# skypilot-org/skypilot

Hardware: AMD Instinct MI355X
Metric: tokens/sec (node) sky-launched Llama-3-8B (higher is better)
Workload: dtype bf16; 1 GPU; model=llama3-8b, global_batch=6, seq_len=4096, parallelism=dp1, sky_launched=True

## Files before the change

skypilot_amd/ops/csrc/attention_bwd.hip:

```cpp
#include <cstdlib>
#include "common.h"

#define ATT_D 128
#define BM 64
#define BN 64

extern "C" __global__ void attn_bwd_pre_kernel(
    const unsigned short* __restrict__ dO, const unsigned short* __restrict__ O,
    float* __restrict__ Dvec, long long rows, int Hq) {
  (void)Hq;
  const int lane = threadIdx.x & 63;
  const long long wave_id =
      (long long)blockIdx.x * (blockDim.x >> 6) + (threadIdx.x >> 6);
  const long long stride = (long long)gridDim.x * (blockDim.x >> 6);
  for (long long row = wave_id; row < rows; row += stride) {
    const unsigned short* drow = dO + row * ATT_D;
    const unsigned short* orow = O + row * ATT_D;
    float acc = bf2f(drow[lane]) * bf2f(orow[lane]) +
                bf2f(drow[lane + 64]) * bf2f(orow[lane + 64]);
    acc = wave_reduce_sum(acc);
    if (lane == 0) Dvec[row] = acc;
  }
}

extern "C" __global__ __launch_bounds__(256, 2) void attn_bwd_dkv_kernel(
    const unsigned short* __restrict__ Q, const unsigned short* __restrict__ K,
    const unsigned short* __restrict__ V, const unsigned short* __restrict__ dO,
    const float* __restrict__ lse, const float* __restrict__ Dvec,
    unsigned short* __restrict__ dK, unsigned short* __restrict__ dV, int B,
    int S, int Hq, int Hkv, float scale, int causal) {
  __shared__ unsigned short q_lds[BM * ATT_D];
  __shared__ unsigned short qt_lds[ATT_D * BM];
  __shared__ unsigned short do_lds[BM * ATT_D];
  __shared__ unsigned short dot_lds[ATT_D * BM];
  __shared__ unsigned short p_lds[BN * BM];
  __shared__ unsigned short ds_lds[BN * BM];
// ... 28 lines not shown
    }
  }

  f32x4 dv_acc[8], dk_acc[8];
#pragma unroll
  for (int ct = 0; ct < 8; ++ct) {
    dv_acc[ct] = f32x4{0.f, 0.f, 0.f, 0.f};
    dk_acc[ct] = f32x4{0.f, 0.f, 0.f, 0.f};
  }

  for (int g = 0; g < group; ++g) {
    const int qh = kvh * group + g;
    const unsigned short* Qb = Q + ((long long)b * S * Hq + qh) * ATT_D;
    const unsigned short* dOb = dO + ((long long)b * S * Hq + qh) * ATT_D;
    const float* lse_b = lse + ((long long)b * Hq + qh) * S;
    const float* dvec_b = Dvec + (long long)b * S * Hq + qh;

    const int qt0 = causal ? kvbase / BM : 0;
    for (int qt = qt0; qt < S / BM; ++qt) {
      const int qbase = qt * BM;
      __syncthreads();
#pragma unroll
      for (int i = 0; i < 4; ++i) {
        int ch = (tid & 7) | ((i & 1) << 3);
        int row = (tid >> 3) | ((i >> 1) << 5);
        s16x8 qv = *(const s16x8*)(Qb + (long long)(qbase + row) * q_rowstride + ch * 8);
        *(s16x8*)((char*)q_lds + swz(row * 256 + ch * 16, row)) = qv;
        s16x8 dov = *(const s16x8*)(dOb + (long long)(qbase + row) * q_rowstride + ch * 8);
        *(s16x8*)((char*)do_lds + swz(row * 256 + ch * 16, row)) = dov;
#pragma unroll
        for (int j = 0; j < 8; ++j) {
// ... 16 lines not shown
          int qrow = ct * 16 + lrow;
          s16x8 bq = *(const s16x8*)((char*)q_lds +
                                     swz(qrow * 256 + (ks * 32 + lgrp * 8) * 2, qrow));
          st[ct] = MFMA_BF16(as_bf16x8(a_k[ks]), as_bf16x8(bq), st[ct]);
          s16x8 bdo = *(const s16x8*)((char*)do_lds +
                                      swz(qrow * 256 + (ks * 32 + lgrp * 8) * 2, qrow));
          dpt[ct] = MFMA_BF16(as_bf16x8(a_v[ks]), as_bf16x8(bdo), dpt[ct]);
        }
      }

      const int my_kvrow = kvbase + 16 * w + lgrp * 4;
#pragma unroll
      for (int ct = 0; ct < 4; ++ct) {
        int qcol = qbase + ct * 16 + lrow;
        float l = lse_b[qcol];
        float dv = dvec_b[(long long)qcol * Hq];
#pragma unroll
        for (int r = 0; r < 4; ++r) {
          float sv = st[ct][r] * scale;
          float pv;
          if ((causal && qcol < my_kvrow + r) || l == -INFINITY)
            pv = 0.f;
          else
            pv = __expf(sv - l);
          int prow = 16 * w + lgrp * 4 + r;
          int pcol = ct * 16 + lrow;
          int off = swzP(prow * 128 + pcol * 2, prow);
          *(unsigned short*)((char*)p_lds + off) = f2bf_trunc(pv);
          *(unsigned short*)((char*)ds_lds + off) =
              f2bf(pv * (dpt[ct][r] - dv));
        }
// ... 54 lines not shown
  const int qbase = qt * BM;

  const int tid = threadIdx.x;
  const int lane = tid & 63;
  const int w = tid >> 6;
  const int lrow = lane & 15;
  const int lgrp = lane >> 4;

  const long long q_rowstride = (long long)Hq * ATT_D;
  const long long kv_rowstride = (long long)Hkv * ATT_D;
  const unsigned short* Qb = Q + ((long long)b * S * Hq + qh) * ATT_D;
  const unsigned short* Kb = K + ((long long)b * S * Hkv + kvh) * ATT_D;
  const unsigned short* Vb = V + ((long long)b * S * Hkv + kvh) * ATT_D;
  const unsigned short* dOb = dO + ((long long)b * S * Hq + qh) * ATT_D;
  const float* lse_b = lse + ((long long)b * Hq + qh) * S;
  const float* dvec_b = Dvec + (long long)b * S * Hq + qh;

  s16x8 a_q[4], a_do[4];
  float my_lse[4], my_dvec[4];
  {
    const int qrow = qbase + 16 * w + lrow;
    const unsigned short* qsrc = Qb + (long long)qrow * q_rowstride;
    const unsigned short* dsrc = dOb + (long long)qrow * q_rowstride;
#pragma unroll
    for (int ks = 0; ks < 4; ++ks) {
      a_q[ks] = *(const s16x8*)(qsrc + ks * 32 + lgrp * 8);
      a_do[ks] = *(const s16x8*)(dsrc + ks * 32 + lgrp * 8);
    }
#pragma unroll
    for (int r = 0; r < 4; ++r) {
      int rr = qbase + 16 * w + lgrp * 4 + r;
      my_lse[r] = lse_b[rr];
      my_dvec[r] = dvec_b[(long long)rr * Hq];
    }
  }

  f32x4 dq_acc[8];
#pragma unroll
  for (int ct = 0; ct < 8; ++ct) dq_acc[ct] = f32x4{0.f, 0.f, 0.f, 0.f};

  const int n_kv_tiles = causal ? (qbase + BM + BN - 1) / BN : S / BN;
  for (int kt = 0; kt < n_kv_tiles; ++kt) {
    const int kvbase = kt * BN;
    __syncthreads();
#pragma unroll
    for (int i = 0; i < 4; ++i) {
      int ch = (tid & 7) | ((i & 1) << 3);
      int row = (tid >> 3) | ((i >> 1) << 5);
// ... 124 lines not shown
  }

  f32x16 dv_acc, dk_acc;
#pragma unroll
  for (int r = 0; r < 16; ++r) {
    dv_acc[r] = 0.f;
    dk_acc[r] = 0.f;
  }

  for (int g = 0; g < group; ++g) {
    const int qh_head = kvh_head * group + g;
    const unsigned short* Qb = Q + ((long long)b * S * Hq + qh_head) * ATT_D;
    const unsigned short* dOb =
        dO + ((long long)b * S * Hq + qh_head) * ATT_D;
    const float* lse_b = lse + ((long long)b * Hq + qh_head) * S;
    const float* dvec_b = Dvec + (long long)b * S * Hq + qh_head;

    const int qt0 = causal ? kvbase / BM : 0;
    for (int qt = qt0; qt < S / BM; ++qt) {
      const int qbase = qt * BM;
      __syncthreads();
#pragma unroll
      for (int i2 = 0; i2 < 2; ++i2) {
        int i = i2 * 2 + (tid >> 8);
        int t = tid & 255;
        int ch = (t & 7) | ((i & 1) << 3);
        int row = (t >> 3) | ((i >> 1) << 5);
        s16x8 qv = *(const s16x8*)(Qb + (long long)(qbase + row) *
                                       q_rowstride + ch * 8);
        *(s16x8*)((char*)q_lds + swz(row * 256 + ch * 16, row)) = qv;
        s16x8 dov = *(const s16x8*)(dOb + (long long)(qbase + row) *
// ... 32 lines not shown
          if ((causal && qcol < kvbase + kvrow) || l == -INFINITY)
            pv = 0.f;
          else
            pv = __expf(acc[r] * scale - l);
          int prow = kvrow;
          int pcol = t_qh * 32 + col;
          *(unsigned short*)((char*)p_lds +
                             swzP(prow * 128 + pcol * 2, prow)) =
              f2bf_trunc(pv);
        }
      }
      __syncthreads();

      if (!is_st) {
        const int qcol = qbase + t_qh * 32 + col;
        const float dvq = dvec_b[(long long)qcol * Hq];
#pragma unroll
        for (int r = 0; r < 16; ++r) {
          int kvrow = t_kvh * 32 + (r & 3) + 8 * (r >> 2) + 4 * half;
          int off = swzP(kvrow * 128 + (t_qh * 32 + col) * 2, kvrow);
          float pv = bf2f(*(const unsigned short*)((char*)p_lds + off));
          *(unsigned short*)((char*)ds_lds + off) =
              f2bf(pv * (acc[r] - dvq));
        }
      }
#pragma unroll
      for (int ks = 0; ks < 4; ++ks) {
        int arow = o_kvh * 32 + col;
        s16x8 afrag = *(const s16x8*)(
            (char*)p_lds +
            swzP(arow * 128 + (ks * 16 + half * 8) * 2, arow));
// ... 29 lines not shown
    dKb[(long long)kvrow * kv_rowstride + d] = f2bf(dk_acc[r] * scale);
    dVb[(long long)kvrow * kv_rowstride + d] = f2bf(dv_acc[r]);
  }
}

extern "C" __global__ void attn_bwd_dkv_tr_kernel(
    const unsigned short*, const unsigned short*, const unsigned short*,
    const unsigned short*, const float*, const float*, unsigned short*,
    unsigned short*, int, int, int, int, float, int);

extern "C" void attn_bwd_v3_launch(const void* Q, const void* K,
                                   const void* V, const void* dO,
                                   const float* lse, const float* Dvec,
                                   void* dQ, void* dK, void* dV, int B,
                                   int S, int Hq, int Hkv, float scale,
                                   bool causal, hipStream_t stream);

extern "C" __global__ void attn_bwd_dkv_swapped_kernel(
    const unsigned short*, const unsigned short*, const unsigned short*,
    const unsigned short*, const float*, const float*, unsigned short*,
    unsigned short*, int, int, int, int, float, int);

extern "C" __global__ void attn_bwd_dq_swapped_kernel(
    const unsigned short*, const unsigned short*, const unsigned short*,
    const unsigned short*, const float*, const float*, unsigned short*,
    int, int, int, int, float, int);

extern "C" void attn_bwd_launch(const void* Q, const void* K, const void* V,
                                const void* O, const void* dO,
                                const float* lse, float* Dvec, void* dQ,
                                void* dK, void* dV, int B, int S, int Hq,
                                int Hkv, float scale, bool causal,
                                hipStream_t stream) {
  long long rows = (long long)B * S * Hq;
  hipLaunchKernelGGL(attn_bwd_pre_kernel, dim3(membound_grid(rows, 4)),
                     dim3(256), 0, stream, (const unsigned short*)dO,
                     (const unsigned short*)O, Dvec, rows, Hq);
  static const int use_bwd_v3 = [] {
    const char* e = getenv("SKY_ATTN_BWD_V3");
    return e ? atoi(e) : 1;
  }();
  if (use_bwd_v3 && S % 128 == 0) {
    attn_bwd_v3_launch(Q, K, V, dO, lse, Dvec, dQ, dK, dV, B, S, Hq, Hkv,
                       scale, causal, stream);
    return;
  }
  static const int dkv_swapped = [] {
    const char* e = getenv("SKY_ATTN_DKV_SWAPPED");
    return e ? atoi(e) : 0;
  }();
  static const int dkv_tr = [] {
    const char* e = getenv("SKY_ATTN_DKV_TR");
    return e ? atoi(e) : 0;
  }();
  if (dkv_tr)
    hipLaunchKernelGGL(attn_bwd_dkv_tr_kernel, dim3(S / BN, B * Hkv),
                       dim3(256), 0, stream, (const unsigned short*)Q,
                       (const unsigned short*)K, (const unsigned short*)V,
                       (const unsigned short*)dO, lse, Dvec,
// ... 51 lines not shown
  const int qbase = qt * BM;

  const int tid = threadIdx.x;
  const int lane = tid & 63;
  const int w = tid >> 6;
  const int lrow = lane & 15;
  const int lgrp = lane >> 4;

  const long long q_rowstride = (long long)Hq * ATT_D;
  const long long kv_rowstride = (long long)Hkv * ATT_D;
  const unsigned short* Qb = Q + ((long long)b * S * Hq + qh) * ATT_D;
  const unsigned short* Kb = K + ((long long)b * S * Hkv + kvh) * ATT_D;
  const unsigned short* Vb = V + ((long long)b * S * Hkv + kvh) * ATT_D;
  const unsigned short* dOb = dO + ((long long)b * S * Hq + qh) * ATT_D;
  const float* lse_b = lse + ((long long)b * Hq + qh) * S;
  const float* dvec_b = Dvec + (long long)b * S * Hq + qh;

  s16x8 q_b[4], do_b[4];
  const int my_q = qbase + 16 * w + lrow;
  {
    const unsigned short* qsrc = Qb + (long long)my_q * q_rowstride;
    const unsigned short* dsrc = dOb + (long long)my_q * q_rowstride;
#pragma unroll
    for (int ks = 0; ks < 4; ++ks) {
      q_b[ks] = *(const s16x8*)(qsrc + ks * 32 + lgrp * 8);
      do_b[ks] = *(const s16x8*)(dsrc + ks * 32 + lgrp * 8);
    }
  }
  const float my_lse = lse_b[my_q];
  const float my_dvec = dvec_b[(long long)my_q * Hq];

  f32x4 dq_t[8];
#pragma unroll
  for (int ct = 0; ct < 8; ++ct) dq_t[ct] = f32x4{0.f, 0.f, 0.f, 0.f};

  const int n_kv_tiles = causal ? (qbase + BM + BN - 1) / BN : S / BN;
  for (int kt = 0; kt < n_kv_tiles; ++kt) {
    const int kvbase = kt * BN;
    __syncthreads();
#pragma unroll
    for (int i = 0; i < 4; ++i) {
      int ch = (tid & 7) | ((i & 1) << 3);
      int row = (tid >> 3) | ((i >> 1) << 5);
      s16x8 kv8 = *(const s16x8*)(Kb + (long long)(kvbase + row) * kv_rowstride + ch * 8);
      *(s16x8*)((char*)k_lds + swz(row * 256 + ch * 16, row)) = kv8;
// ... 117 lines not shown
    }
  }

  f32x4 dv_t[8], dk_t[8];
#pragma unroll
  for (int ct = 0; ct < 8; ++ct) {
    dv_t[ct] = f32x4{0.f, 0.f, 0.f, 0.f};
    dk_t[ct] = f32x4{0.f, 0.f, 0.f, 0.f};
  }

  for (int g = 0; g < group; ++g) {
    const int qh = kvh * group + g;
    const unsigned short* Qb = Q + ((long long)b * S * Hq + qh) * ATT_D;
    const unsigned short* dOb = dO + ((long long)b * S * Hq + qh) * ATT_D;
    const float* lse_b = lse + ((long long)b * Hq + qh) * S;
    const float* dvec_b = Dvec + (long long)b * S * Hq + qh;

    const int qt0 = causal ? kvbase / BM : 0;
    for (int qt = qt0; qt < S / BM; ++qt) {
      const int qbase = qt * BM;
      __syncthreads();
#pragma unroll
      for (int i = 0; i < 4; ++i) {
        int ch = (tid & 7) | ((i & 1) << 3);
        int row = (tid >> 3) | ((i >> 1) << 5);
        s16x8 qv = *(const s16x8*)(Qb + (long long)(qbase + row) * q_rowstride + ch * 8);
        *(s16x8*)((char*)q_lds + swz(row * 256 + ch * 16, row)) = qv;
        s16x8 dov = *(const s16x8*)(dOb + (long long)(qbase + row) * q_rowstride + ch * 8);
        *(s16x8*)((char*)do_lds + swz(row * 256 + ch * 16, row)) = dov;
#pragma unroll
        for (int j = 0; j < 8; ++j) {
// ... 20 lines not shown
          s16x8 a_q = *(const s16x8*)((char*)q_lds +
              swz(qrow * 256 + (ks * 32 + lgrp * 8) * 2, qrow));
          sp[qsub] = MFMA_BF16(as_bf16x8(a_q), as_bf16x8(k_b[ks]),
                               sp[qsub]);
          s16x8 a_do = *(const s16x8*)((char*)do_lds +
              swz(qrow * 256 + (ks * 32 + lgrp * 8) * 2, qrow));
          dp[qsub] = MFMA_BF16(as_bf16x8(a_do), as_bf16x8(v_b[ks]),
                               dp[qsub]);
        }

      float lse_l[4], dv_l[4];
#pragma unroll
      for (int qsub = 0; qsub < 4; ++qsub) {
        int qc = qbase + qsub * 16 + lrow;
        lse_l[qsub] = lse_b[qc];
        dv_l[qsub] = dvec_b[(long long)qc * Hq];
      }
#pragma unroll
      for (int qsub = 0; qsub < 4; ++qsub)
#pragma unroll
        for (int r = 0; r < 4; ++r) {
          int qrow = qbase + qsub * 16 + lgrp * 4 + r;
          float l = __shfl(lse_l[qsub], lgrp * 4 + r, 64);
          float pv;
          if ((causal && qrow < my_kv) || l == -INFINITY)
            pv = 0.f;
          else
            pv = __expf(sp[qsub][r] * scale - l);
          sp[qsub][r] = pv;
          dp[qsub][r] = pv * (dp[qsub][r] -
                              __shfl(dv_l[qsub], lgrp * 4 + r, 64));
// ... 90 lines not shown
  f32x4 dv_acc[8], dk_acc[8];
#pragma unroll
  for (int ct = 0; ct < 8; ++ct) {
    dv_acc[ct] = f32x4{0.f, 0.f, 0.f, 0.f};
    dk_acc[ct] = f32x4{0.f, 0.f, 0.f, 0.f};
  }

  const unsigned int q_base_a = (unsigned int)(unsigned long long)q_lds;
  const unsigned int do_base_a = (unsigned int)(unsigned long long)do_lds;

  for (int g = 0; g < group; ++g) {
    const int qh = kvh * group + g;
    const unsigned short* Qb = Q + ((long long)b * S * Hq + qh) * ATT_D;
    const unsigned short* dOb = dO + ((long long)b * S * Hq + qh) * ATT_D;
    const float* lse_b = lse + ((long long)b * Hq + qh) * S;
    const float* dvec_b = Dvec + (long long)b * S * Hq + qh;

    const int qt0 = causal ? kvbase / BM : 0;
    for (int qt = qt0; qt < S / BM; ++qt) {
      const int qbase = qt * BM;
      __syncthreads();
#pragma unroll
      for (int i = 0; i < 4; ++i) {
        int idx = tid + i * 256;
        int row = idx >> 4, ch = idx & 15;
        s16x8 qv = *(const s16x8*)(Qb + (long long)(qbase + row) * q_rowstride + ch * 8);
        *(s16x8*)((char*)q_lds + swz(row * 256 + ch * 16, row)) = qv;
        s16x8 dov = *(const s16x8*)(dOb + (long long)(qbase + row) * q_rowstride + ch * 8);
        *(s16x8*)((char*)do_lds + swz(row * 256 + ch * 16, row)) = dov;
      }
      __syncthreads();
// ... 8 lines not shown
          int qrow = ct * 16 + lrow;
          s16x8 bq = *(const s16x8*)((char*)q_lds +
                                     swz(qrow * 256 + (ks * 32 + lgrp * 8) * 2, qrow));
          st[ct] = MFMA_BF16(as_bf16x8(a_k[ks]), as_bf16x8(bq), st[ct]);
          s16x8 bdo = *(const s16x8*)((char*)do_lds +
                                      swz(qrow * 256 + (ks * 32 + lgrp * 8) * 2, qrow));
          dpt[ct] = MFMA_BF16(as_bf16x8(a_v[ks]), as_bf16x8(bdo), dpt[ct]);
        }
      }

      const int my_kvrow = kvbase + 16 * w + lgrp * 4;
#pragma unroll
      for (int ct = 0; ct < 4; ++ct) {
        int qcol = qbase + ct * 16 + lrow;
        float l = lse_b[qcol];
        float dvv = dvec_b[(long long)qcol * Hq];
#pragma unroll
        for (int r = 0; r < 4; ++r) {
          float sv = st[ct][r] * scale;
          float pv;
          if ((causal && qcol < my_kvrow + r) || l == -INFINITY)
            pv = 0.f;
          else
            pv = __expf(sv - l);
          int prow = 16 * w + lgrp * 4 + r;
          int pcol = ct * 16 + lrow;
          int off = swzP(prow * 128 + pcol * 2, prow);
          *(unsigned short*)((char*)p_lds + off) = f2bf_trunc(pv);
          *(unsigned short*)((char*)ds_lds + off) =
              f2bf(pv * (dpt[ct][r] - dvv));
        }
// ... 71 lines not shown
```

skypilot_amd/ops/csrc/attention_bwd_v3.hip:

```cpp
#include <cstdlib>

#include "attn_v3.h"

#define ATT_D 128

__device__ __forceinline__ int vsubz(int q, int d) {
  return (((q >> 2) << 3) + ((d >> 4) ^ ((q >> 2) & 7))) * 64 +
         ((q & 3) << 4) + (d & 15);
}

extern "C" __global__ __launch_bounds__(256, 2) void attn_bwd_dkv_v3_kernel(
    const unsigned short* __restrict__ Q, const unsigned short* __restrict__ K,
    const unsigned short* __restrict__ V, const unsigned short* __restrict__ dO,
    const float* __restrict__ lse, const float* __restrict__ Dvec,
    unsigned short* __restrict__ dK, unsigned short* __restrict__ dV, int B,
    int S, int Hq, int Hkv, float scale, int causal) {
  __shared__ unsigned short q_lds[32 * ATT_D];
  __shared__ unsigned short do_lds[32 * ATT_D];
  __shared__ unsigned short k_own[128 * ATT_D];
  __shared__ unsigned short v_own[128 * ATT_D];

  const int kt = blockIdx.x;
  const int bh = blockIdx.y;
  const int b = bh / Hkv;
// ... 39 lines not shown
  for (int dt = 0; dt < 4; ++dt)
#pragma unroll
    for (int r = 0; r < 16; ++r) {
      dv_acc[dt][r] = 0.f;
      dk_acc[dt][r] = 0.f;
    }

  const int qt0 = causal ? kvb / 32 : 0;
  const int n_qt = S / 32;

  for (int gi = 0; gi < group; ++gi) {
    const int qh = kvh * group + gi;
    const unsigned short* Qb = Q + ((long long)b * S * Hq + qh) * ATT_D;
    const unsigned short* dOb = dO + ((long long)b * S * Hq + qh) * ATT_D;
    const float* lse_b = lse + ((long long)b * Hq + qh) * S;
    const float* dvec_b = Dvec + (long long)b * S * Hq + qh;

    for (int qt = qt0; qt < n_qt; ++qt) {
      const int qbase = qt * 32;
      __syncthreads();
#pragma unroll
      for (int i = 0; i < 2; ++i) {
        int c = tid * 2 + i;
        int qr = c >> 4;
        int dch = (c & 15) * 8;
        long long src = (long long)(qbase + qr) * q_rowstride + dch;
        int off = qr * 256 + (((dch >> 3) ^ (qr & 15)) << 4);
        *(s16x8*)((char*)q_lds + off) = *(const s16x8*)(Qb + src);
        *(s16x8*)((char*)do_lds + off) = *(const s16x8*)(dOb + src);
      }
      __syncthreads();
// ... 21 lines not shown
            swzK16((32 * w + col) * 256 + (ks * 2 + h) * 16, 32 * w + col));
        dpt = MFMA32V3(as_bf16x8(ad), as_bf16x8(vfr), dpt);
      }
      __builtin_amdgcn_s_setprio(0);

      const bool need_mask = causal && qbase < kvb + 128;
#pragma unroll
      for (int r = 0; r < 16; ++r) {
        const int ql = (r & 3) + ((r >> 2) << 3) + (h << 2);
        float lv = lse_b[qbase + ql];
        float l2 = (lv == -INFINITY) ? 3.0e37f
                                     : lv * 1.44269504088896340736f;
        float p = exp2f(st[r] - l2);
        if (need_mask && qbase + ql < my_kv) p = 0.f;
        st[r] = p;
        dpt[r] = p * (dpt[r] - dvec_b[(long long)(qbase + ql) * Hq]);
      }

      s16x8 pa, da;
      tr4 t0, t1;
#define DKV_TRA(base, qv, dv)                                             \
  ((base) + (qv) * 256 + ((((dv) >> 3) ^ ((qv) & 15)) << 4) +             \
   (((dv) & 7) << 1))
#define DKV_TR_ISSUE(lds_base, ks)                                        \
  {                                                                       \
    int q_s = (ks) * 16 + ((g >> 1) << 3) + (lw >> 2);                    \
    int d_s = ((g & 1) << 4) + ((lw & 3) << 2);                           \
    unsigned base = (unsigned)(size_t)((char*)(lds_base));                \
    ds_tr4_issue(&t0, DKV_TRA(base, q_s, d_s),                            \
                 DKV_TRA(base, q_s + 4, d_s),                             \
                 DKV_TRA(base, q_s, 32 + d_s),                            \
// ... 43 lines not shown
  unsigned short* dKb = dK + ((long long)b * S * Hkv + kvh) * ATT_D;
  unsigned short* dVb = dV + ((long long)b * S * Hkv + kvh) * ATT_D;
#pragma unroll
  for (int r = 0; r < 16; ++r) {
    const int kvrow = kvb + 32 * w + (r & 3) + ((r >> 2) << 3) + (h << 2);
    unsigned short* krow = dKb + (long long)kvrow * kv_rowstride;
    unsigned short* vrow = dVb + (long long)kvrow * kv_rowstride;
#pragma unroll
    for (int dt = 0; dt < 4; ++dt) {
      krow[dt * 32 + col] = f2bf(dk_acc[dt][r] * scale);
      vrow[dt * 32 + col] = f2bf(dv_acc[dt][r]);
    }
  }
}

extern "C" __global__ __launch_bounds__(256, 2) void attn_bwd_dq_v3_kernel(
    const unsigned short* __restrict__ Q, const unsigned short* __restrict__ K,
    const unsigned short* __restrict__ V, const unsigned short* __restrict__ dO,
    const float* __restrict__ lse, const float* __restrict__ Dvec,
    unsigned short* __restrict__ dQ, int B, int S, int Hq, int Hkv,
    float scale, int causal) {
  __shared__ unsigned short k_lds[2][64 * ATT_D];
  __shared__ unsigned short v_lds[2][64 * ATT_D];

  const int nq = S / 128;
  const bool paired = causal && (int)gridDim.x * 2 == nq;
  const int qtA = paired ? nq - 1 - (int)blockIdx.x
                         : (int)gridDim.x - 1 - (int)blockIdx.x;
  const int qtB = paired ? (int)blockIdx.x : 0;
  const int bh = blockIdx.y;
// ... 22 lines not shown
  s16x8 q_b[8];
  float lse2, dvq;
#define DQ_LOAD_Q()                                                       \
  {                                                                       \
    const float qs = scale * 1.44269504088896340736f;                     \
    const unsigned short* src = Qb + (long long)my_q * q_rowstride;       \
    _Pragma("unroll") for (int ks = 0; ks < 8; ++ks) {                    \
      s16x8 raw = *(const s16x8*)(src + ks * 16 + h * 8);                 \
      _Pragma("unroll") for (int j = 0; j < 8; ++j)                       \
        raw[j] = (short)f2bf(bf2f((unsigned short)raw[j]) * qs);          \
      q_b[ks] = raw;                                                      \
    }                                                                     \
    float lv = lse[((long long)b * Hq + qh) * S + my_q];                  \
    lse2 = (lv == -INFINITY) ? 3.0e37f                                    \
                             : lv * 1.44269504088896340736f;              \
    dvq = Dvec[((long long)b * S + my_q) * Hq + qh];                      \
  }
  DQ_LOAD_Q();
  const unsigned short* do_src = dOb + (long long)my_q * q_rowstride;

  f32x16 dq_acc[4];
#pragma unroll
  for (int dt = 0; dt < 4; ++dt)
#pragma unroll
    for (int r = 0; r < 16; ++r) dq_acc[dt][r] = 0.f;

  const int nt_A = causal ? (qbase + 128) / 64 : S / 64;
  const int nt_B = paired ? (qtB * 128 + 128) / 64 : 0;
  const int total_t = nt_A + nt_B;
  int w_tiles = causal ? ((qbase + 32 * w + 31) >> 6) + 1 : nt_A;

// ... 161 lines not shown
    V3_PACK2(db, dpt, 3);
    lgkm_wait0_bind2(&t0, &t1);
    DQ_MFMA(db);
  }

  DQ_EPILOGUE();
#undef DQ_EPILOGUE
#undef DQ_LOAD_Q
}

extern "C" void attn_bwd_v3_launch(const void* Q, const void* K,
                                   const void* V, const void* dO,
                                   const float* lse, const float* Dvec,
                                   void* dQ, void* dK, void* dV, int B,
                                   int S, int Hq, int Hkv, float scale,
                                   bool causal, hipStream_t stream) {
  dim3 gkv(S / 128, B * Hkv);
  hipLaunchKernelGGL(attn_bwd_dkv_v3_kernel, gkv, dim3(256), 0, stream,
                     (const unsigned short*)Q, (const unsigned short*)K,
                     (const unsigned short*)V, (const unsigned short*)dO,
                     lse, Dvec, (unsigned short*)dK, (unsigned short*)dV, B,
                     S, Hq, Hkv, scale, causal ? 1 : 0);
  int nqq = S / 128;
  int gqx = (causal && nqq % 2 == 0) ? nqq / 2 : nqq;
  dim3 gq(gqx, B * Hq);
  hipLaunchKernelGGL(attn_bwd_dq_v3_kernel, gq, dim3(256), 0, stream,
                     (const unsigned short*)Q, (const unsigned short*)K,
                     (const unsigned short*)V, (const unsigned short*)dO,
                     lse, Dvec, (unsigned short*)dQ, B, S, Hq, Hkv, scale,
                     causal ? 1 : 0);
}
```

skypilot_amd/ops/csrc/attn_v3.h:

```cpp
#pragma once
#include "common.h"

typedef __attribute__((ext_vector_type(16))) float f32x16;
#define MFMA32V3(a, b, c) \
  __builtin_amdgcn_mfma_f32_32x32x16_bf16(a, b, c, 0, 0, 0)

__device__ __forceinline__ int swzK16(int byte_off, int row) {
  return byte_off ^ ((row & 15) << 4);
}

__device__ __forceinline__ int vsub(int kv, int d) {
  return (((kv >> 2) << 3) + (d >> 4)) * 64 + ((kv & 3) << 4) + (d & 15);
}

__device__ __forceinline__ unsigned cvtpk_bf16(float a, float b) {
  unsigned r;
  asm volatile("v_cvt_pk_bf16_f32 %0, %1, %2" : "=v"(r) : "v"(a), "v"(b));
  return r;
}

__device__ __forceinline__ float xhalf32(float x) {
  union { float f; unsigned u; } c;
  c.f = x;
  auto p = __builtin_amdgcn_permlane32_swap(c.u, c.u, false, false);
// ... 14 lines not shown
}
__device__ __forceinline__ void vm_drain() {
  asm volatile("s_waitcnt vmcnt(0)" ::: "memory");
}

__device__ __forceinline__ void lgkm_wait0_bind2(tr4* a, tr4* b) {
  asm volatile("s_waitcnt lgkmcnt(0)"
               : "+v"(a->d[0]), "+v"(a->d[1]), "+v"(a->d[2]),
                 "+v"(a->d[3]), "+v"(b->d[0]), "+v"(b->d[1]),
                 "+v"(b->d[2]), "+v"(b->d[3])
               :
               : "memory");
  __builtin_amdgcn_sched_barrier(0);
}

__device__ __forceinline__ void gload_lds16(const void* g, void* l) {
  __builtin_amdgcn_global_load_lds(
      (const __attribute__((address_space(1))) unsigned int*)g,
      (__attribute__((address_space(3))) unsigned int*)l, 16, 0, 0);
}


#define V3_PACK_CORE(pb, c0, c1, c2, c3, c4, c5, c6, c7)                  \
  {                                                                       \
    unsigned w0a = cvtpk_bf16(c0, c1);                                    \
    unsigned w1a = cvtpk_bf16(c2, c3);                                    \
    unsigned w0b = cvtpk_bf16(c4, c5);                                    \
    unsigned w1b = cvtpk_bf16(c6, c7);                                    \
    auto p0 = __builtin_amdgcn_permlane32_swap(w0a, w0b, false, false);   \
    auto p1 = __builtin_amdgcn_permlane32_swap(w1a, w1b, false, false);   \
// ... 23 lines not shown
```

skypilot_amd/ops/csrc/bindings.cpp:

```cpp
#include <torch/extension.h>

#include <ATen/hip/HIPContext.h>
#include <hip/hip_runtime.h>

#include <vector>

#define CHECK_GPU(x) TORCH_CHECK(x.is_cuda(), #x " must be on GPU")
#define CHECK_CONTIG(x) TORCH_CHECK(x.is_contiguous(), #x " must be contiguous")
#define CHECK_BF16(x) \
  TORCH_CHECK(x.scalar_type() == at::kBFloat16, #x " must be bf16")

static hipStream_t cur_stream() {
  return at::hip::getCurrentHIPStream().stream();
}

extern "C" {
void rmsnorm_fwd_launch(const void*, const void*, void*, float*, long long,
                        int, float, hipStream_t);
void rmsnorm_bwd_launch(const void*, const void*, const void*, const float*,
                        void*, float*, long long, int, hipStream_t);
void rope_launch(const void*, void*, const float*, const float*, const int*,
                 long long, int, int, bool, hipStream_t);
void adamw_launch(void*, float*, const void*, float*, float*, long long,
                  float, float, float, float, float, int, float, hipStream_t);
void cross_entropy_launch(void*, const int*, float*, long long, int, float,
                          int, hipStream_t);
void attn_fwd_launch(const void*, const void*, const void*, void*, float*,
                     int, int, int, int, float, bool, hipStream_t);
void attn_bwd_launch(const void*, const void*, const void*, const void*,
                     const void*, const float*, float*, void*, void*, void*,
                     int, int, int, int, float, bool, hipStream_t);
void mfma_probe_launch(const void*, const void*, float*, hipStream_t);
void mfma32_probe_launch(const void*, const void*, float*, hipStream_t);
void trb16_probe_launch(float*, int, hipStream_t);
void permlane_probe_launch(float*, hipStream_t);
void skinny_gemm_launch(const void*, const void*, void*, int, int, int,
                        hipStream_t);
void skinny_gemm_swiglu_launch(const void*, const void*, void*, int, int,
                               int, hipStream_t);
void transpose_bf16_launch(const void*, void*, int, int, hipStream_t);
void skinny_gemm_fp8_launch(const void*, const float*, const void*, void*,
                            int, int, int, hipStream_t);
void gemm_nt_launch(const void*, const void*, void*, int, int, long long,
                    hipStream_t);
void adamw_mt_launch(const void*, const void*, const void*, const void*,
                     const void*, long long, float, float, float, float,
// ... 107 lines not shown
  const int Hkv = (int)K.size(2);
  TORCH_CHECK(D == 128, "attention kernel requires head_dim=128");
  TORCH_CHECK(S % 64 == 0, "seq len must be a multiple of 64");
  TORCH_CHECK(Hq % Hkv == 0);
  auto O = torch::empty_like(Q);
  auto lse = torch::empty({B, Hq, S}, Q.options().dtype(at::kFloat));
  attn_fwd_launch(Q.data_ptr(), K.data_ptr(), V.data_ptr(), O.data_ptr(),
                  lse.data_ptr<float>(), B, S, Hq, Hkv, (float)scale, causal,
                  cur_stream());
  return {O, lse};
}

std::vector<torch::Tensor> attn_bwd(torch::Tensor Q, torch::Tensor K,
                                    torch::Tensor V, torch::Tensor O,
                                    torch::Tensor dO, torch::Tensor lse,
                                    double scale, bool causal) {
  CHECK_GPU(Q); CHECK_CONTIG(dO);
  const int B = (int)Q.size(0), S = (int)Q.size(1), Hq = (int)Q.size(2);
  const int Hkv = (int)K.size(2);
  auto dQ = torch::empty_like(Q);
  auto dK = torch::empty_like(K);
  auto dV = torch::empty_like(V);
  auto Dvec = torch::empty({(long)B * S * Hq}, Q.options().dtype(at::kFloat));
  attn_bwd_launch(Q.data_ptr(), K.data_ptr(), V.data_ptr(), O.data_ptr(),
                  dO.data_ptr(), lse.data_ptr<float>(),
                  Dvec.data_ptr<float>(), dQ.data_ptr(), dK.data_ptr(),
                  dV.data_ptr(), B, S, Hq, Hkv, (float)scale, causal,
                  cur_stream());
  return {dQ, dK, dV};
}

torch::Tensor attn_decode(torch::Tensor Q, torch::Tensor Kc,
                          torch::Tensor Vc, torch::Tensor kv_lens,
                          torch::Tensor slot_ids, double scale) {
  CHECK_GPU(Q); CHECK_CONTIG(Q); CHECK_BF16(Q);
  TORCH_CHECK(kv_lens.scalar_type() == at::kInt);
  TORCH_CHECK(slot_ids.scalar_type() == at::kInt);
  const int B = (int)Q.size(0), Hq = (int)Q.size(1), D = (int)Q.size(2);
  const int S_max = (int)Kc.size(1), Hkv = (int)Kc.size(2);
  TORCH_CHECK(D == 128);
  auto O = torch::empty_like(Q);
  attn_decode_launch(Q.data_ptr(), Kc.data_ptr(), Vc.data_ptr(),
                     O.data_ptr(), kv_lens.data_ptr<int>(),
// ... 251 lines not shown
}

torch::Tensor permlane_probe(torch::Tensor ref_dev) {
  auto out = torch::zeros({64, 2}, ref_dev.options().dtype(at::kFloat));
  permlane_probe_launch(out.data_ptr<float>(), cur_stream());
  return out;
}

PYBIND11_MODULE(TORCH_EXTENSION_NAME, m) {
  m.def("rmsnorm_fwd", &rmsnorm_fwd);
  m.def("rmsnorm_bwd", &rmsnorm_bwd);
  m.def("rope", &rope);
  m.def("adamw_step", &adamw_step);
  m.def("cross_entropy_fused", &cross_entropy_fused);
  m.def("attn_fwd", &attn_fwd);
  m.def("attn_bwd", &attn_bwd);
  m.def("attn_decode", &attn_decode);
  m.def("skinny_gemm", &skinny_gemm);
  m.def("skinny_gemm_fp8", &skinny_gemm_fp8);
  m.def("transpose_bf16", &transpose_bf16);
  m.def("gemm_nt", &gemm_nt);
  m.def("wgrad_tn", &wgrad_tn);
  m.def("adamw_step_mt", &adamw_step_mt);
  m.def("skinny_gemm_swiglu", &skinny_gemm_swiglu);
  m.def("rmsnorm_res", &rmsnorm_res);
  m.def("rope_kvwrite", &rope_kvwrite);
  m.def("decode_advance", &decode_advance);
  m.def("attn_decode_qkv", &attn_decode_qkv);
  m.def("skinny_gemm_fp8_norm", &skinny_gemm_fp8_norm);
  m.def("swiglu_fwd", &swiglu_fwd);
  m.def("swiglu_bwd", &swiglu_bwd);
// ... 6 lines not shown
```

Before: 19000 tokens/s.

## Add pipelined dK/dV backward kernel with head-major Dvec and heavy-first grid

Changes the Dvec layout from [B,S,H] to [B,H,S] so per-head reads in every backward kernel become contiguous and can be vector-loaded. Adds a new dK/dV kernel that keeps a 128-row K/V tile in LDS with the softmax scale pre-folded into K. It register-prefetches the next Q/dO tile across the (group, q-tile) loop, uses transposed LDS reads with immediate offsets and MFMA scheduling hints. The default variant swaps grid axes so heavy causal tiles launch first. This adds more LDS use, extra code paths selectable by env or argument, and a rounding change from pre-scaling K in bf16.

```diff
diff --git a/skypilot_amd/ops/csrc/attention_bwd.hip b/skypilot_amd/ops/csrc/attention_bwd.hip
--- a/skypilot_amd/ops/csrc/attention_bwd.hip
+++ b/skypilot_amd/ops/csrc/attention_bwd.hip
@@ -7,8 +7,7 @@
 
 extern "C" __global__ void attn_bwd_pre_kernel(
     const unsigned short* __restrict__ dO, const unsigned short* __restrict__ O,
-    float* __restrict__ Dvec, long long rows, int Hq) {
-  (void)Hq;
+    float* __restrict__ Dvec, long long rows, int S, int Hq) {
   const int lane = threadIdx.x & 63;
   const long long wave_id =
       (long long)blockIdx.x * (blockDim.x >> 6) + (threadIdx.x >> 6);
@@ -19,7 +18,11 @@
     float acc = bf2f(drow[lane]) * bf2f(orow[lane]) +
                 bf2f(drow[lane + 64]) * bf2f(orow[lane + 64]);
     acc = wave_reduce_sum(acc);
-    if (lane == 0) Dvec[row] = acc;
+    const int hh = (int)(row % Hq);
+    const long long bs = row / Hq;
+    const int ss = (int)(bs % S);
+    const long long bb = bs / S;
+    if (lane == 0) Dvec[(bb * Hq + hh) * S + ss] = acc;
   }
 }
 
@@ -78,7 +81,7 @@
     const unsigned short* Qb = Q + ((long long)b * S * Hq + qh) * ATT_D;
     const unsigned short* dOb = dO + ((long long)b * S * Hq + qh) * ATT_D;
     const float* lse_b = lse + ((long long)b * Hq + qh) * S;
-    const float* dvec_b = Dvec + (long long)b * S * Hq + qh;
+    const float* dvec_b = Dvec + ((long long)b * Hq + qh) * S;
 
     const int qt0 = causal ? kvbase / BM : 0;
     for (int qt = qt0; qt < S / BM; ++qt) {
@@ -125,7 +128,7 @@
       for (int ct = 0; ct < 4; ++ct) {
         int qcol = qbase + ct * 16 + lrow;
         float l = lse_b[qcol];
-        float dv = dvec_b[(long long)qcol * Hq];
+        float dv = dvec_b[qcol];
 #pragma unroll
         for (int r = 0; r < 4; ++r) {
           float sv = st[ct][r] * scale;
@@ -210,7 +213,7 @@
   const unsigned short* Vb = V + ((long long)b * S * Hkv + kvh) * ATT_D;
   const unsigned short* dOb = dO + ((long long)b * S * Hq + qh) * ATT_D;
   const float* lse_b = lse + ((long long)b * Hq + qh) * S;
-  const float* dvec_b = Dvec + (long long)b * S * Hq + qh;
+  const float* dvec_b = Dvec + ((long long)b * Hq + qh) * S;
 
   s16x8 a_q[4], a_do[4];
   float my_lse[4], my_dvec[4];
@@ -227,7 +230,7 @@
     for (int r = 0; r < 4; ++r) {
       int rr = qbase + 16 * w + lgrp * 4 + r;
       my_lse[r] = lse_b[rr];
-      my_dvec[r] = dvec_b[(long long)rr * Hq];
+      my_dvec[r] = dvec_b[rr];
     }
   }
 
@@ -382,7 +385,7 @@
     const unsigned short* dOb =
         dO + ((long long)b * S * Hq + qh_head) * ATT_D;
     const float* lse_b = lse + ((long long)b * Hq + qh_head) * S;
-    const float* dvec_b = Dvec + (long long)b * S * Hq + qh_head;
+    const float* dvec_b = Dvec + ((long long)b * Hq + qh_head) * S;
 
     const int qt0 = causal ? kvbase / BM : 0;
     for (int qt = qt0; qt < S / BM; ++qt) {
@@ -445,7 +448,7 @@
 
       if (!is_st) {
         const int qcol = qbase + t_qh * 32 + col;
-        const float dvq = dvec_b[(long long)qcol * Hq];
+        const float dvq = dvec_b[qcol];
 #pragma unroll
         for (int r = 0; r < 16; ++r) {
           int kvrow = t_kvh * 32 + (r & 3) + 8 * (r >> 2) + 4 * half;
@@ -505,7 +508,8 @@
                                    const float* lse, const float* Dvec,
                                    void* dQ, void* dK, void* dV, int B,
                                    int S, int Hq, int Hkv, float scale,
-                                   bool causal, hipStream_t stream);
+                                   bool causal, int dkv_variant,
+                                   hipStream_t stream);
 
 extern "C" __global__ void attn_bwd_dkv_swapped_kernel(
     const unsigned short*, const unsigned short*, const unsigned short*,
@@ -522,18 +526,18 @@
                                 const float* lse, float* Dvec, void* dQ,
                                 void* dK, void* dV, int B, int S, int Hq,
                                 int Hkv, float scale, bool causal,
-                                hipStream_t stream) {
+                                int dkv_variant, hipStream_t stream) {
   long long rows = (long long)B * S * Hq;
   hipLaunchKernelGGL(attn_bwd_pre_kernel, dim3(membound_grid(rows, 4)),
                      dim3(256), 0, stream, (const unsigned short*)dO,
-                     (const unsigned short*)O, Dvec, rows, Hq);
+                     (const unsigned short*)O, Dvec, rows, S, Hq);
   static const int use_bwd_v3 = [] {
     const char* e = getenv("SKY_ATTN_BWD_V3");
     return e ? atoi(e) : 1;
   }();
-  if (use_bwd_v3 && S % 128 == 0) {
+  if ((use_bwd_v3 || dkv_variant >= 0) && S % 128 == 0) {
     attn_bwd_v3_launch(Q, K, V, dO, lse, Dvec, dQ, dK, dV, B, S, Hq, Hkv,
-                       scale, causal, stream);
+                       scale, causal, dkv_variant, stream);
     return;
   }
   static const int dkv_swapped = [] {
@@ -615,7 +619,7 @@
   const unsigned short* Vb = V + ((long long)b * S * Hkv + kvh) * ATT_D;
   const unsigned short* dOb = dO + ((long long)b * S * Hq + qh) * ATT_D;
   const float* lse_b = lse + ((long long)b * Hq + qh) * S;
-  const float* dvec_b = Dvec + (long long)b * S * Hq + qh;
+  const float* dvec_b = Dvec + ((long long)b * Hq + qh) * S;
 
   s16x8 q_b[4], do_b[4];
   const int my_q = qbase + 16 * w + lrow;
@@ -629,7 +633,7 @@
     }
   }
   const float my_lse = lse_b[my_q];
-  const float my_dvec = dvec_b[(long long)my_q * Hq];
+  const float my_dvec = dvec_b[my_q];
 
   f32x4 dq_t[8];
 #pragma unroll
@@ -777,7 +781,7 @@
     const unsigned short* Qb = Q + ((long long)b * S * Hq + qh) * ATT_D;
     const unsigned short* dOb = dO + ((long long)b * S * Hq + qh) * ATT_D;
     const float* lse_b = lse + ((long long)b * Hq + qh) * S;
-    const float* dvec_b = Dvec + (long long)b * S * Hq + qh;
+    const float* dvec_b = Dvec + ((long long)b * Hq + qh) * S;
 
     const int qt0 = causal ? kvbase / BM : 0;
     for (int qt = qt0; qt < S / BM; ++qt) {
@@ -828,7 +832,7 @@
       for (int qsub = 0; qsub < 4; ++qsub) {
         int qc = qbase + qsub * 16 + lrow;
         lse_l[qsub] = lse_b[qc];
-        dv_l[qsub] = dvec_b[(long long)qc * Hq];
+        dv_l[qsub] = dvec_b[qc];
       }
 #pragma unroll
       for (int qsub = 0; qsub < 4; ++qsub)
@@ -949,7 +953,7 @@
     const unsigned short* Qb = Q + ((long long)b * S * Hq + qh) * ATT_D;
     const unsigned short* dOb = dO + ((long long)b * S * Hq + qh) * ATT_D;
     const float* lse_b = lse + ((long long)b * Hq + qh) * S;
-    const float* dvec_b = Dvec + (long long)b * S * Hq + qh;
+    const float* dvec_b = Dvec + ((long long)b * Hq + qh) * S;
 
     const int qt0 = causal ? kvbase / BM : 0;
     for (int qt = qt0; qt < S / BM; ++qt) {
@@ -988,7 +992,7 @@
       for (int ct = 0; ct < 4; ++ct) {
         int qcol = qbase + ct * 16 + lrow;
         float l = lse_b[qcol];
-        float dvv = dvec_b[(long long)qcol * Hq];
+        float dvv = dvec_b[qcol];
 #pragma unroll
         for (int r = 0; r < 4; ++r) {
           float sv = st[ct][r] * scale;
diff --git a/skypilot_amd/ops/csrc/attention_bwd_v3.hip b/skypilot_amd/ops/csrc/attention_bwd_v3.hip
--- a/skypilot_amd/ops/csrc/attention_bwd_v3.hip
+++ b/skypilot_amd/ops/csrc/attention_bwd_v3.hip
@@ -77,7 +77,7 @@
     const unsigned short* Qb = Q + ((long long)b * S * Hq + qh) * ATT_D;
     const unsigned short* dOb = dO + ((long long)b * S * Hq + qh) * ATT_D;
     const float* lse_b = lse + ((long long)b * Hq + qh) * S;
-    const float* dvec_b = Dvec + (long long)b * S * Hq + qh;
+    const float* dvec_b = Dvec + ((long long)b * Hq + qh) * S;
 
     for (int qt = qt0; qt < n_qt; ++qt) {
       const int qbase = qt * 32;
@@ -129,7 +129,7 @@
         float p = exp2f(st[r] - l2);
         if (need_mask && qbase + ql < my_kv) p = 0.f;
         st[r] = p;
-        dpt[r] = p * (dpt[r] - dvec_b[(long long)(qbase + ql) * Hq]);
+        dpt[r] = p * (dpt[r] - dvec_b[qbase + ql]);
       }
 
       s16x8 pa, da;
@@ -203,6 +203,239 @@
   }
 }
 
+typedef const __attribute__((address_space(1))) char* gptr_t;
+__device__ __forceinline__ gptr_t uniform_ptr(const void* p) {
+  const unsigned long long v = (unsigned long long)p;
+  const unsigned lo = __builtin_amdgcn_readfirstlane((unsigned)v);
+  const unsigned hi = __builtin_amdgcn_readfirstlane((unsigned)(v >> 32));
+  return (gptr_t)(((unsigned long long)hi << 32) | lo);
+}
+typedef const __attribute__((address_space(1))) s16x8* g_s16x8_t;
+typedef const __attribute__((address_space(1))) f32x4* g_f32x4_t;
+
+extern "C" __global__ __launch_bounds__(256, 2) void attn_bwd_dkv_v3p_kernel(
+    const unsigned short* __restrict__ Q, const unsigned short* __restrict__ K,
+    const unsigned short* __restrict__ V, const unsigned short* __restrict__ dO,
+    const float* __restrict__ lse, const float* __restrict__ Dvec,
+    unsigned short* __restrict__ dK, unsigned short* __restrict__ dV, int B,
+    int S, int Hq, int Hkv, float scale, int causal, int heavy_first) {
+  __shared__ unsigned short lds[(2 * 32 + 2 * 128) * ATT_D];
+  unsigned short* q_lds = lds;
+  unsigned short* do_lds = lds + 32 * ATT_D;
+  unsigned short* k_own = lds + 64 * ATT_D;
+  unsigned short* v_own = lds + 192 * ATT_D;
+
+  const int kt = heavy_first ? blockIdx.y : blockIdx.x;
+  const int bh = heavy_first ? blockIdx.x : blockIdx.y;
+  const int b = bh / Hkv;
+  const int kvh = bh % Hkv;
+  const int group = Hq / Hkv;
+  const int kvb = kt * 128;
+
+  const int tid = threadIdx.x;
+  const int lane = tid & 63;
+  const int w = tid >> 6;
+  const int col = lane & 31;
+  const int h = lane >> 5;
+  const int g = lane >> 4;
+  const int lw = lane & 15;
+
+  const long long q_rowstride = (long long)Hq * ATT_D;
+  const long long kv_rowstride = (long long)Hkv * ATT_D;
+  const unsigned short* Kb = K + ((long long)b * S * Hkv + kvh) * ATT_D;
+  const unsigned short* Vb = V + ((long long)b * S * Hkv + kvh) * ATT_D;
+
+  const int my_kv = kvb + 32 * w + col;
+
+  const int qt0 = causal ? kvb / 32 : 0;
+  const int n_qt = S / 32;
+
+  unsigned tra[8];
+  {
+    const int q_s = ((g >> 1) << 3) + (lw >> 2);
+    const int d_s = ((g & 1) << 4) + ((lw & 3) << 2);
+    const unsigned base = (unsigned)(size_t)((char*)q_lds);
+#pragma unroll
+    for (int i = 0; i < 8; ++i)
+      tra[i] = DKV_TRA(base, q_s + 4 * (i & 1), 32 * (i >> 1) + d_s);
+  }
+#define DKVP_TR_ISSUE(off)                                                \
+  {                                                                       \
+    ds_tr4_issue_off<(off)>(&t0, tra[0], tra[1], tra[2], tra[3]);         \
+    ds_tr4_issue_off<(off)>(&t1, tra[4], tra[5], tra[6], tra[7]);         \
+  }
+
+  const unsigned frag_q = (unsigned)swzK16(col * 256 + h * 16, col);
+  const unsigned frag_k = frag_q + (unsigned)w * 8192u;
+
+  s16x8 pq[2], pd[2];
+  const unsigned st_off =
+      (unsigned)(((tid * 2) >> 4) * q_rowstride + ((tid * 2) & 15) * 8) * 2u;
+  const unsigned row_off = (unsigned)h * 16u;
+#define DKVP_PREFETCH(qh_, qbase_)                                        \
+  {                                                                       \
+    const long long tb = ((long long)b * S * Hq + (qh_)) * ATT_D +        \
+                         (long long)(qbase_) * q_rowstride;               \
+    gptr_t qsrc = uniform_ptr(Q + tb) + st_off;                           \
+    gptr_t dsrc = uniform_ptr(dO + tb) + st_off;                          \
+    _Pragma("unroll") for (int i = 0; i < 2; ++i) {                       \
+      pq[i] = *(g_s16x8_t)(qsrc + 16 * i);                                \
+      pd[i] = *(g_s16x8_t)(dsrc + 16 * i);                                \
+    }                                                                     \
+  }
+  DKVP_PREFETCH(kvh * group, qt0 * 32);
+
+  const float ksc = scale * 1.44269504088896340736f;
+  {
+#pragma unroll
+    for (int i = 0; i < 8; ++i) {
+      int c = tid * 8 + i;
+      int kr = c >> 4;
+      int dch = (c & 15) * 8;
+      long long src = (long long)(kvb + kr) * kv_rowstride + dch;
+      s16x8 raw = *(const s16x8*)(Kb + src);
+#pragma unroll
+      for (int j = 0; j < 8; ++j)
+        raw[j] = (short)f2bf(bf2f((unsigned short)raw[j]) * ksc);
+      int koff = kr * 256 + (((dch >> 3) ^ (kr & 15)) << 4);
+      *(s16x8*)((char*)k_own + koff) = raw;
+      *(s16x8*)((char*)v_own + koff) = *(const s16x8*)(Vb + src);
+    }
+  }
+
+  f32x16 dv_acc[4], dk_acc[4];
+#pragma unroll
+  for (int dt = 0; dt < 4; ++dt)
+#pragma unroll
+    for (int r = 0; r < 16; ++r) {
+      dv_acc[dt][r] = 0.f;
+      dk_acc[dt][r] = 0.f;
+    }
+
+  for (int gi = 0; gi < group; ++gi) {
+    const int qh = kvh * group + gi;
+    const float* lse_b = lse + ((long long)b * Hq + qh) * S;
+    const float* dvec_b = Dvec + ((long long)b * Hq + qh) * S;
+
+    for (int qt = qt0; qt < n_qt; ++qt) {
+      const int qbase = qt * 32;
+      f32x4 lv4[4], dv4[4];
+      gptr_t lse_t = uniform_ptr(lse_b + qbase);
+      gptr_t dvec_t = uniform_ptr(dvec_b + qbase);
+#pragma unroll
+      for (int j = 0; j < 4; ++j) {
+        lv4[j] = *(g_f32x4_t)(lse_t + 32 * j + row_off);
+        dv4[j] = *(g_f32x4_t)(dvec_t + 32 * j + row_off);
+      }
+      __syncthreads();
+#pragma unroll
+      for (int i = 0; i < 2; ++i) {
+        int c = tid * 2 + i;
+        int qr = c >> 4;
+        int dch = (c & 15) * 8;
+        int off = qr * 256 + (((dch >> 3) ^ (qr & 15)) << 4);
+        *(s16x8*)((char*)q_lds + off) = pq[i];
+        *(s16x8*)((char*)do_lds + off) = pd[i];
+      }
+      __syncthreads();
+      {
+        int nqt = qt + 1, ngi = gi;
+        if (nqt == n_qt) {
+          nqt = qt0;
+          ngi = gi + 1;
+        }
+        if (ngi == group) {
+          nqt = qt;
+          ngi = gi;
+        }
+        DKVP_PREFETCH(kvh * group + ngi, nqt * 32);
+      }
+      if (causal && qbase + 31 < kvb + 32 * w) {
+#pragma unroll
+        for (int j = 0; j < 4; ++j)
+          asm volatile("" ::"v"(lv4[j]), "v"(dv4[j]));
+        continue;
+      }
+
+      f32x16 st, dpt;
+#pragma unroll
+      for (int r = 0; r < 16; ++r) {
+        st[r] = 0.f;
+        dpt[r] = 0.f;
+      }
+      unsigned fq = frag_q, fk = frag_k;
+      asm volatile("" : "+v"(fq), "+v"(fk));
+      __builtin_amdgcn_s_setprio(1);
+#pragma unroll
+      for (int ks = 0; ks < 8; ++ks) {
+        const unsigned oq = fq ^ (ks << 5), ok = fk ^ (ks << 5);
+        s16x8 aq = *(const s16x8*)((char*)q_lds + oq);
+        s16x8 kfr = *(const s16x8*)((char*)k_own + ok);
+        st = MFMA32V3(as_bf16x8(aq), as_bf16x8(kfr), st);
+        s16x8 ad = *(const s16x8*)((char*)do_lds + oq);
+        s16x8 vfr = *(const s16x8*)((char*)v_own + ok);
+        dpt = MFMA32V3(as_bf16x8(ad), as_bf16x8(vfr), dpt);
+      }
+      __builtin_amdgcn_sched_group_barrier(0x100, 4, 0);
+#pragma unroll
+      for (int i = 0; i < 14; ++i) {
+        __builtin_amdgcn_sched_group_barrier(0x008, 1, 0);
+        __builtin_amdgcn_sched_group_barrier(0x100, 2, 0);
+      }
+      __builtin_amdgcn_sched_group_barrier(0x008, 2, 0);
+      __builtin_amdgcn_s_setprio(0);
+
+      const bool need_mask = causal && qbase < kvb + 128;
+#pragma unroll
+      for (int r = 0; r < 16; ++r) {
+        const int ql = (r & 3) + ((r >> 2) << 3) + (h << 2);
+        float lv = lv4[r >> 2][r & 3];
+        float l2 = (lv == -INFINITY) ? 3.0e37f
+                                     : lv * 1.44269504088896340736f;
+        float p = exp2f(st[r] - l2);
+        if (need_mask && qbase + ql < my_kv) p = 0.f;
+        st[r] = p;
+        dpt[r] = p * (dpt[r] - dv4[r >> 2][r & 3]);
+      }
+
+      s16x8 pa, da;
+      tr4 t0, t1;
+      DKVP_TR_ISSUE(8192);
+      V3_PACK1(pa, st, 0);
+      lgkm_wait0_bind2(&t0, &t1);
+      DKV_MFMA(dv_acc, pa);
+      DKVP_TR_ISSUE(8192 + 4096);
+      V3_PACK1(pa, st, 1);
+      lgkm_wait0_bind2(&t0, &t1);
+      DKV_MFMA(dv_acc, pa);
+      DKVP_TR_ISSUE(0);
+      V3_PACK1(da, dpt, 0);
+      lgkm_wait0_bind2(&t0, &t1);
+      DKV_MFMA(dk_acc, da);
+      DKVP_TR_ISSUE(4096);
+      V3_PACK1(da, dpt, 1);
+      lgkm_wait0_bind2(&t0, &t1);
+      DKV_MFMA(dk_acc, da);
+    }
+  }
+#undef DKVP_PREFETCH
+#undef DKVP_TR_ISSUE
+
+  unsigned short* dKb = dK + ((long long)b * S * Hkv + kvh) * ATT_D;
+  unsigned short* dVb = dV + ((long long)b * S * Hkv + kvh) * ATT_D;
+#pragma unroll
+  for (int r = 0; r < 16; ++r) {
+    const int kvrow = kvb + 32 * w + (r & 3) + ((r >> 2) << 3) + (h << 2);
+    unsigned short* krow = dKb + (long long)kvrow * kv_rowstride;
+    unsigned short* vrow = dVb + (long long)kvrow * kv_rowstride;
+#pragma unroll
+    for (int dt = 0; dt < 4; ++dt) {
+      krow[dt * 32 + col] = f2bf(dk_acc[dt][r] * scale);
+      vrow[dt * 32 + col] = f2bf(dv_acc[dt][r]);
+    }
+  }
+}
+
 extern "C" __global__ __launch_bounds__(256, 2) void attn_bwd_dq_v3_kernel(
     const unsigned short* __restrict__ Q, const unsigned short* __restrict__ K,
     const unsigned short* __restrict__ V, const unsigned short* __restrict__ dO,
@@ -255,7 +488,7 @@
     float lv = lse[((long long)b * Hq + qh) * S + my_q];                  \
     lse2 = (lv == -INFINITY) ? 3.0e37f                                    \
                              : lv * 1.44269504088896340736f;              \
-    dvq = Dvec[((long long)b * S + my_q) * Hq + qh];                      \
+    dvq = Dvec[((long long)b * Hq + qh) * S + my_q];                      \
   }
   DQ_LOAD_Q();
   const unsigned short* do_src = dOb + (long long)my_q * q_rowstride;
@@ -447,13 +680,30 @@
                                    const float* lse, const float* Dvec,
                                    void* dQ, void* dK, void* dV, int B,
                                    int S, int Hq, int Hkv, float scale,
-                                   bool causal, hipStream_t stream) {
-  dim3 gkv(S / 128, B * Hkv);
-  hipLaunchKernelGGL(attn_bwd_dkv_v3_kernel, gkv, dim3(256), 0, stream,
-                     (const unsigned short*)Q, (const unsigned short*)K,
-                     (const unsigned short*)V, (const unsigned short*)dO,
-                     lse, Dvec, (unsigned short*)dK, (unsigned short*)dV, B,
-                     S, Hq, Hkv, scale, causal ? 1 : 0);
+                                   bool causal, int dkv_variant,
+                                   hipStream_t stream) {
+  static const int dkv_env = [] {
+    const char* e = getenv("SKY_ATTN_DKV_PIPE");
+    const int v = e ? atoi(e) : 2;
+    return v < 0 || v > 2 ? 2 : v;
+  }();
+  const int variant = dkv_variant >= 0 ? dkv_variant : dkv_env;
+  if (variant == 0) {
+    dim3 gkv(S / 128, B * Hkv);
+    hipLaunchKernelGGL(attn_bwd_dkv_v3_kernel, gkv, dim3(256), 0, stream,
+                       (const unsigned short*)Q, (const unsigned short*)K,
+                       (const unsigned short*)V, (const unsigned short*)dO,
+                       lse, Dvec, (unsigned short*)dK, (unsigned short*)dV,
+                       B, S, Hq, Hkv, scale, causal ? 1 : 0);
+  } else {
+    const int heavy_first = variant == 2 ? 1 : 0;
+    dim3 gkv = heavy_first ? dim3(B * Hkv, S / 128) : dim3(S / 128, B * Hkv);
+    hipLaunchKernelGGL(attn_bwd_dkv_v3p_kernel, gkv, dim3(256), 0, stream,
+                       (const unsigned short*)Q, (const unsigned short*)K,
+                       (const unsigned short*)V, (const unsigned short*)dO,
+                       lse, Dvec, (unsigned short*)dK, (unsigned short*)dV,
+                       B, S, Hq, Hkv, scale, causal ? 1 : 0, heavy_first);
+  }
   int nqq = S / 128;
   int gqx = (causal && nqq % 2 == 0) ? nqq / 2 : nqq;
   dim3 gq(gqx, B * Hq);
diff --git a/skypilot_amd/ops/csrc/attn_v3.h b/skypilot_amd/ops/csrc/attn_v3.h
--- a/skypilot_amd/ops/csrc/attn_v3.h
+++ b/skypilot_amd/ops/csrc/attn_v3.h
@@ -52,6 +52,21 @@
   __builtin_amdgcn_sched_barrier(0);
 }
 
+template <int OFF>
+__device__ __forceinline__ void ds_tr4_issue_off(tr4* t, unsigned a0,
+                                                 unsigned a1, unsigned a2,
+                                                 unsigned a3) {
+  static_assert(OFF >= 0 && OFF < 65536, "DS offset field is 16 bits");
+  asm volatile(
+      "ds_read_b64_tr_b16 %0, %4 offset:%8\n\t"
+      "ds_read_b64_tr_b16 %1, %5 offset:%8\n\t"
+      "ds_read_b64_tr_b16 %2, %6 offset:%8\n\t"
+      "ds_read_b64_tr_b16 %3, %7 offset:%8"
+      : "=v"(t->d[0]), "=v"(t->d[1]), "=v"(t->d[2]), "=v"(t->d[3])
+      : "v"(a0), "v"(a1), "v"(a2), "v"(a3), "n"(OFF)
+      : "memory");
+}
+
 __device__ __forceinline__ void gload_lds16(const void* g, void* l) {
   __builtin_amdgcn_global_load_lds(
       (const __attribute__((address_space(1))) unsigned int*)g,
diff --git a/skypilot_amd/ops/csrc/bindings.cpp b/skypilot_amd/ops/csrc/bindings.cpp
--- a/skypilot_amd/ops/csrc/bindings.cpp
+++ b/skypilot_amd/ops/csrc/bindings.cpp
@@ -29,7 +29,7 @@
                      int, int, int, int, float, bool, hipStream_t);
 void attn_bwd_launch(const void*, const void*, const void*, const void*,
                      const void*, const float*, float*, void*, void*, void*,
-                     int, int, int, int, float, bool, hipStream_t);
+                     int, int, int, int, float, bool, int, hipStream_t);
 void mfma_probe_launch(const void*, const void*, float*, hipStream_t);
 void mfma32_probe_launch(const void*, const void*, float*, hipStream_t);
 void trb16_probe_launch(float*, int, hipStream_t);
@@ -167,8 +167,11 @@
 std::vector<torch::Tensor> attn_bwd(torch::Tensor Q, torch::Tensor K,
                                     torch::Tensor V, torch::Tensor O,
                                     torch::Tensor dO, torch::Tensor lse,
-                                    double scale, bool causal) {
+                                    double scale, bool causal,
+                                    int64_t dkv_variant) {
   CHECK_GPU(Q); CHECK_CONTIG(dO);
+  TORCH_CHECK(dkv_variant >= -1 && dkv_variant <= 2,
+              "attn_bwd: dkv_variant must be -1, 0, 1 or 2");
   const int B = (int)Q.size(0), S = (int)Q.size(1), Hq = (int)Q.size(2);
   const int Hkv = (int)K.size(2);
   auto dQ = torch::empty_like(Q);
@@ -179,7 +182,7 @@
                   dO.data_ptr(), lse.data_ptr<float>(),
                   Dvec.data_ptr<float>(), dQ.data_ptr(), dK.data_ptr(),
                   dV.data_ptr(), B, S, Hq, Hkv, (float)scale, causal,
-                  cur_stream());
+                  (int)dkv_variant, cur_stream());
   return {dQ, dK, dV};
 }
 
@@ -461,7 +464,9 @@
   m.def("adamw_step", &adamw_step);
   m.def("cross_entropy_fused", &cross_entropy_fused);
   m.def("attn_fwd", &attn_fwd);
-  m.def("attn_bwd", &attn_bwd);
+  m.def("attn_bwd", &attn_bwd, py::arg("Q"), py::arg("K"), py::arg("V"),
+        py::arg("O"), py::arg("dO"), py::arg("lse"), py::arg("scale"),
+        py::arg("causal"), py::arg("dkv_variant") = -1);
   m.def("attn_decode", &attn_decode);
   m.def("skinny_gemm", &skinny_gemm);
   m.def("skinny_gemm_fp8", &skinny_gemm_fp8);
```

Measured after the change: 20380 tokens/s, median of 6. 7.2% higher.
